# dke-lab/dgll

Hardware: AMD Instinct MI355X
Metric: aggregated edges/sec + epoch time, 3-layer GraphSAGE ogbn-products, 1/2/4/8 GPU (higher is better)
Workload: dtype bf16

## Files before the change

dgll_amd/_lib.py:

```python
import contextlib
import ctypes as C
import os

import torch

_HERE = os.path.dirname(os.path.abspath(__file__))
LIB_PATH = os.path.join(_HERE, "lib", "libdgll_hip.so")

OK = 0
F32, BF16 = 0, 1
REDUCE_SUM, REDUCE_MEAN = 0, 1
EPI_NONE, EPI_BIAS, EPI_RELU = 0, 1, 2


class BatchLoad(C.Structure):
    _fields_ = [("staged_host", C.c_void_p), ("staged_entries", C.c_int64), ("staged_dev", C.c_void_p),
                ("pos_host", C.c_void_p), ("n_outer", C.c_int64), ("pos_bytes", C.c_int), ("pos_dev", C.c_void_p),
                ("indptr", C.c_void_p), ("indices", C.c_void_p),
                ("n_hops", C.c_int), ("rows", C.c_int64 * 8), ("seeds_off", C.c_int64), ("src_off", C.c_int64 * 8), ("ptr_off", C.c_int64 * 8),
                ("cache", C.c_void_p), ("ldc", C.c_int64), ("host", C.c_void_p), ("ldh", C.c_int64), ("slot", C.c_void_p),
                ("host_map", C.c_void_p), ("feat", C.c_int), ("dtype", C.c_int), ("miss_count", C.c_void_p),
                ("feat_out", C.c_void_p * 8), ("ld_feat", C.c_int64),
                ("reduced_out", C.c_void_p), ("ld_reduced", C.c_int64), ("reduce", C.c_int),
                ("ids_out", C.c_void_p),
# ... 45 lines not shown
        _build.build()
    if not os.path.exists(LIB_PATH):
        raise ImportError("libdgll_hip.so is missing (expected at %s); run `python -m dgll_amd.build`" % LIB_PATH)
    return C.CDLL(LIB_PATH)


lib = _load()

_vp, _i32, _i64, _sz = C.c_void_p, C.c_int, C.c_int64, C.c_size_t

SIGNATURES = {
    "dgll_hip_abi_version": (_i32, []),
    "dgll_hip_last_error": (C.c_char_p, []),
    "dgll_hip_device_info": (_i32, [_i32, C.c_char_p, _i32, C.POINTER(_i32), C.POINTER(_i64)]),
    "dgll_hip_debug_tune": (_i32, [_i32, _i32]),
    "dgll_hip_debug_spmm_choice": (_i32, [_i32, _i32, _i32, _i64, _i32, _i64, _i64, _i64, _i32, _i32, _i32, _i32, _i32, _vp]),
    "dgll_hip_debug_gat_choice": (_i32, [_i32] * 17 + [_i64, _i32, _i64, _i64, _i64, _i64, _i32, _vp]),
    "dgll_hip_debug_transform_choice": (_i32, [_i32] * 12 + [_i64, _i32, _vp]),
    "dgll_hip_csr_plan_create": (_i32, [_vp, _vp, _i64, _i64, _i32, C.POINTER(_vp)]),
    "dgll_hip_csr_plan_destroy": (None, [_vp]),
    "dgll_hip_csr_plan_workspace_bytes": (_sz, [_vp, _i32]),
    "dgll_hip_csr_plan_num_long_rows": (_i64, [_vp]),
    "dgll_hip_csr_plan_num_chunks": (_i64, [_vp]),
    "dgll_hip_spmm_csr": (_i32, [_vp, _vp, _vp, _vp, _vp, _vp, _i64, _i32, _vp, _i64, _i32, _i64, _i64, _i32, _i32,
                                 _i32, _vp, _vp, _sz]),
    "dgll_hip_spmm_csr_ex": (_i32, [_vp, _vp, _vp, _vp, _vp, _vp, _i64, _i32, _vp, _i64, _i32, _i64, _i64, _i32, _i32,
                                    _i32, _vp, _vp, _sz, _vp, _i32]),
    "dgll_hip_spmm_csr_gated": (_i32, [_vp, _vp, _vp, _vp, _vp, _vp, _i64, _i32, _vp, _i64, _i32, _i64, _i64, _i32, _i32,
                                       _i32, _vp, _vp, _sz, _vp, _i32, _vp, _i64]),
    "dgll_hip_sage_fused_forward": (_i32, [_vp, _vp, _vp, _vp, _vp, _vp, _i64, _i32, _i32, _vp, _i64, _i32, _vp, _i64, _vp, _i64, _i32,
                                           _vp, _i32, _vp, _i64, _i32, _vp, _i64, _i64, _i64, _vp, _sz]),
    "dgll_hip_sddmm_csr": (_i32, [_vp, _vp, _vp, _vp, _i64, _vp, _i64, _i32, _vp, _i64, _i32]),
    "dgll_hip_gat_fwd": (_i32, [_vp, _vp, _vp, _vp, _vp, _i64, _vp, _vp, _vp, _vp, _i64, _i32, _vp, _vp, _i64, _i32, _i32,
                                C.c_float, _i32, _i32, _vp, _sz]),
    "dgll_hip_gat_fwd_ex": (_i32, [_vp, _vp, _vp, _vp, _vp, _i64, _vp, _vp, _vp, _vp, _i64, _i32, _vp, _i64, _i32, _i32,
                                   C.c_float, _i32, _vp, _sz, _i32, _i32]),
    "dgll_hip_gat_bwd_rows": (_i32, [_vp, _vp, _vp, _vp, _vp, _i64, _vp, _vp, _vp, _vp, _i64, _vp, _i64, _i32, _vp, _vp, _vp,
                                     _i64, _vp, _vp, _i64, _i32, _i32, C.c_float, _i32, _i32, _i32, _vp, _sz]),
    "dgll_hip_gat_bwd_rows_split": (_i32, [_vp, _vp, _vp, _vp, _vp, _i64, _vp, _vp, _vp, _i64, _vp, _i64, _i32, _vp, _vp, _i64, _vp, _vp,
                                           _i64, _i32, _i32, C.c_float, _i32, _i32, _vp, _vp, _sz]),
    "dgll_hip_gat_bwd_cols": (_i32, [_vp, _vp, _vp, _vp, _vp, _vp, _i64, _vp, _i64, _vp, _vp, _vp, _vp, _vp, _vp, _i64, _vp,
                                     _i32, _i64, _i32, _i32, C.c_float, _i32, _vp, _sz]),
    "dgll_hip_gat_fwd_strided": (_i32, [_vp, _vp, _vp, _vp, _vp, _i64, _vp, _vp, _i32, _vp, _i64, _i32, _vp, _i64, _i32, _i32,
                                        C.c_float, _i32, _vp, _sz]),
    "dgll_host_sampler_pool_create": (_i32, [_vp, _vp, _vp, _vp, _i64, _i64, _vp, _vp, _i32, C.c_uint64, C.c_uint64, _i32, _i32, _vp, _i64,
                                             _i64, _vp, _vp, _vp, _i32]),
# ... 206 lines not shown
```

dgll_amd/csrc/common.hpp:

```cpp
#pragma once
#include <hip/hip_runtime.h>

#include "host_common.hpp"

struct dgll_csr_plan {
    int device = 0;
    int64_t n_rows = 0, nnz = 0;
    int threshold = 256;
    int64_t n_long = 0, n_chunks = 0;
    int64_t* d_long_row = nullptr;
    int32_t* d_long_chunk0 = nullptr;
    int64_t* d_chunk_begin = nullptr;
    int64_t* d_chunk_end = nullptr;
    int64_t* d_chunk_row = nullptr;
    int flat_edges = 0;
    int64_t n_flat = 0;
    int64_t* d_flat_row0 = nullptr;
};

namespace dgll {

constexpr int kWave = 64;
constexpr int kBlock = 256;
constexpr int kWavesPerBlock = kBlock / kWave;
constexpr int kXcds = 8;

typedef uint16_t bf16_t;
typedef __attribute__((ext_vector_type(2))) __bf16 bf16x2_t;
typedef __attribute__((ext_vector_type(2))) float f32x2_t;

int hip_fail(hipError_t e, const char* what);

#define DGLL_HIP_TRY(expr)                                          \
    do {                                                            \
        hipError_t _e = (expr);                                     \
        if (_e != hipSuccess) return ::dgll::hip_fail(_e, #expr);   \
    } while (0)
// ... 106 lines not shown
```

dgll_amd/csrc/spmm.hip:

```cpp
#include <algorithm>
#include <vector>

#include "common.hpp"
#include "gat_choice.hpp"
#include "gather.hpp"
#include <type_traits>

namespace dgll {

struct LongRow { int64_t row, begin, end; };

__global__ void find_long_rows_kernel(const int64_t* __restrict__ rowptr, int64_t n_rows, int threshold,
                                      LongRow* __restrict__ out, unsigned long long* __restrict__ count,
                                      unsigned long long capacity) {
    for (int64_t r = blockIdx.x * (int64_t)blockDim.x + threadIdx.x; r < n_rows; r += (int64_t)gridDim.x * blockDim.x) {
        const int64_t b = rowptr[r], e = rowptr[r + 1];
        if (e - b > threshold) {
            const unsigned long long at = atomicAdd(count, 1ull);
            if (at < capacity) out[at] = LongRow{r, b, e};
        }
    }
}

constexpr int64_t kFlatRowCost = 4;
// ... 1 lines not shown
                                 int64_t* __restrict__ row0) {
    for (int64_t w = blockIdx.x * (int64_t)blockDim.x + threadIdx.x; w <= n_flat; w += (int64_t)gridDim.x * blockDim.x) {
        if (w == n_flat) { row0[w] = n_rows; continue; }
        const int64_t target = w * cost_per_wave;
        int64_t lo = 0, hi = n_rows;
        while (lo < hi) {
            const int64_t mid = (lo + hi) >> 1;
            if (rowptr[mid] + kFlatRowCost * mid < target) lo = mid + 1; else hi = mid;
        }
        row0[w] = lo;
    }
}

struct SpmmArgs {
    const int64_t* rowptr;
    const int32_t* col;
    const float* val;
    const void* X;
    void* Y;
    int64_t ldx, ldy, n_rows;
    int feat, reduce, epilogue;
    const float* bias;
    int threshold;
    int64_t n_chunks;
    const int64_t* chunk_begin;
    const int64_t* chunk_end;
    float* ws;
    int ws_ld;
    uint32_t chunk_blocks, row_blocks;
    int rows_per_wave;
    int flags;
    const float* row_scale;
    int accumulate;
    const void* gate;
    int64_t ldg;
    const int64_t* flat_row0;
    int64_t n_flat;
};

constexpr int kSpmmXcdRemap = 1;
constexpr int kSpmmAligned16 = 2;
constexpr int kSpmmPrefetchNext = 4;

template <typename T> __device__ __forceinline__ float load_one(const T* p);
template <> __device__ __forceinline__ float load_one<float>(const float* p) { return *p; }
template <> __device__ __forceinline__ float load_one<bf16_t>(const bf16_t* p) { return bf16_to_f32(*p); }

// ... 94 lines not shown
}

template <typename L> __device__ __forceinline__ float spmm_row_scale(const SpmmArgs& a, int64_t row, L len) {
    return a.row_scale ? a.row_scale[row] : ((a.reduce == DGLL_REDUCE_MEAN && len > 0) ? 1.0f / (float)len : 1.0f);
}

template <typename YT, int EPV, bool EXTRA, typename L>
__device__ __forceinline__ void spmm_finish_row(const SpmmArgs& a, int64_t row, L len, int c0, float (&acc)[EPV]) {
    YT* yrow = static_cast<YT*>(a.Y) + row * a.ldy;
    const bool full = c0 + EPV <= a.feat;
    RowVec<YT, EPV> prev, gatev;
    const YT* grow = nullptr;
    if constexpr (EXTRA) {
        grow = a.gate ? static_cast<const YT*>(a.gate) + row * a.ldg : nullptr;
        if (full) {
            if (a.accumulate) prev.load(yrow + c0);
            if (grow) gatev.load(grow + c0);
        }
    }
    finish_row<YT, EPV, EXTRA>(yrow, c0, a.feat, spmm_row_scale(a, row, len), a.epilogue, a.bias, acc, a.accumulate, grow, full, prev,
                               gatev);
}

template <typename XT, int EPV, int LPR, bool HAS_VAL, int U>
__device__ __forceinline__ void spmm_chunk_item(const SpmmArgs& a, const XT* __restrict__ xcol, int c0, bool col_ok, int lane, int wave,
                                                uint32_t bid) {
    const int64_t chunk = __builtin_amdgcn_readfirstlane((int)(bid * kWavesPerBlock + wave));
    if (chunk >= a.n_chunks) return;
    float acc[EPV];
#pragma unroll
    for (int i = 0; i < EPV; ++i) acc[i] = 0.0f;
    gather_edges<XT, EPV, LPR, HAS_VAL, U>(a.col, a.val, xcol, a.ldx, uniform64(a.chunk_begin[chunk]), uniform64(a.chunk_end[chunk]),
                                           lane, acc);
    if (lane < LPR && col_ok) {
        float* w = a.ws + chunk * a.ws_ld + c0;
#pragma unroll
        for (int i = 0; i < EPV; ++i) w[i] = acc[i];
    }
}

template <typename XT, typename YT, int EPV, int LPR, bool HAS_VAL, int U, bool EXTRA, bool PF = false>
__global__ __launch_bounds__(kBlock) void spmm_csr_kernel(const SpmmArgs a) {
    const int lane = lane_id();
    const int wave = __builtin_amdgcn_readfirstlane((int)(threadIdx.x >> 6));
    const int sub = lane % LPR;
    const int c0 = ((int)blockIdx.y * LPR + sub) * EPV;
    const bool col_ok = c0 < a.feat;
    const XT* xcol = static_cast<const XT*>(a.X) + (col_ok ? c0 : 0);
    uint32_t bid = blockIdx.x;

    if (bid < a.chunk_blocks) { spmm_chunk_item<XT, EPV, LPR, HAS_VAL, U>(a, xcol, c0, col_ok, lane, wave, bid); return; }

    bid -= a.chunk_blocks;
    if (a.flags & kSpmmXcdRemap) bid = xcd_remap(bid, a.row_blocks);
    const int64_t row0 = ((int64_t)bid * kWavesPerBlock + wave) * a.rows_per_wave;
    constexpr bool pf = PF;
    int64_t nb_ = 0, ne_ = 0;
    int ncol = 0;
    float nval = 0.0f;
    if (pf && row0 < a.n_rows) {
        nb_ = uniform64(a.rowptr[row0]); ne_ = uniform64(a.rowptr[row0 + 1]);
        if (nb_ + lane < ne_) {
            ncol = __builtin_nontemporal_load(a.col + nb_ + lane);
            if (HAS_VAL) nval = __builtin_nontemporal_load(a.val + nb_ + lane);
        }
    }
    for (int r = 0; r < a.rows_per_wave; ++r) {
        const int64_t row = row0 + r;
        if (row >= a.n_rows) return;
        int64_t b, e;
        int fcol = 0;
        float fval = 0.0f;
        if (pf) {
            b = nb_; e = ne_; fcol = ncol; fval = nval;
// ... 12 lines not shown
        if constexpr (EXTRA) {
            if (a.accumulate == 2 && e == b) continue;
        }
        float acc[EPV];
#pragma unroll
        for (int i = 0; i < EPV; ++i) acc[i] = 0.0f;
        gather_edges<XT, EPV, LPR, HAS_VAL, U>(a.col, a.val, xcol, a.ldx, b, e, lane, acc, pf, fcol, fval);
        if (lane < LPR && col_ok) spmm_finish_row<YT, EPV, EXTRA>(a, row, e - b, c0, acc);
    }
}

template <typename XT, typename YT, int EPV, int LPR, bool HAS_VAL, int U, bool EXTRA>
__global__ __launch_bounds__(kBlock) void spmm_csr_flat_kernel(const SpmmArgs a) {
    typedef VecIO<XT, EPV> IO;
    constexpr int SLOTS = kWave / LPR, G = SLOTS * U;
    const int lane = lane_id();
    const int wave = __builtin_amdgcn_readfirstlane((int)(threadIdx.x >> 6));
    const int sub = lane % LPR, slot = lane / LPR;
    const int c0 = ((int)blockIdx.y * LPR + sub) * EPV;
    const bool col_ok = c0 < a.feat;
    const XT* xcol = static_cast<const XT*>(a.X) + (col_ok ? c0 : 0);
    uint32_t bid = blockIdx.x;

    if (bid < a.chunk_blocks) { spmm_chunk_item<XT, EPV, LPR, HAS_VAL, U>(a, xcol, c0, col_ok, lane, wave, bid); return; }
    bid -= a.chunk_blocks;
    const int64_t w = (int64_t)bid * kWavesPerBlock + wave;
    if (w >= a.n_flat) return;
    int64_t r = uniform64(a.flat_row0[w]);
    const int64_t r_end = uniform64(a.flat_row0[w + 1]);
    if (r >= r_end) return;
    int64_t rb = uniform64(a.rowptr[r]), re = uniform64(a.rowptr[r + 1]);
    const int64_t p_end = uniform64(a.rowptr[r_end]);
    int64_t p = rb;
    const bool writer = lane < LPR && col_ok;
    const uint32_t ld32 = (uint32_t)a.ldx;
    const int thr = a.threshold;
    float acc[EPV];
#pragma unroll
    for (int i = 0; i < EPV; ++i) acc[i] = 0.0f;
    bool stop = false;

    auto flush = [&]() {
#pragma unroll
        for (int off = LPR; off < kWave; off <<= 1) {
#pragma unroll
            for (int i = 0; i < EPV; ++i) acc[i] += __shfl_xor(acc[i], off);
        }
// ... 105 lines not shown
            j += cnt;
            if (q0 + cnt == re) {
                flush();
                while (!stop && re == rb) flush();
            }
        }
        p = stop ? rb : p + j;
    }
}

template <typename XT, typename YT, int EPV, int LPR, bool HAS_VAL, bool EXTRA>
__global__ __launch_bounds__(kBlock) void spmm_rowslot_kernel(const SpmmArgs a) {
    typedef VecIO<XT, EPV> IO;
    constexpr int SLOTS = kWave / LPR;
    constexpr int U = 4;
    const int lane = lane_id();
    const int wave = __builtin_amdgcn_readfirstlane((int)(threadIdx.x >> 6));
    const int sub = lane % LPR, slot = lane / LPR;
    const int c0 = ((int)blockIdx.y * LPR + sub) * EPV;
    const bool col_ok = c0 < a.feat;
    const XT* xcol = static_cast<const XT*>(a.X) + (col_ok ? c0 : 0);
    uint32_t bid = blockIdx.x;

    if (bid < a.chunk_blocks) { spmm_chunk_item<XT, EPV, LPR, HAS_VAL, U>(a, xcol, c0, col_ok, lane, wave, bid); return; }
    bid -= a.chunk_blocks;
    const uint32_t ld32 = (uint32_t)a.ldx;
    const int64_t row0 = ((int64_t)bid * kWavesPerBlock + wave) * a.rows_per_wave;
    for (int r = 0; r < a.rows_per_wave; r += SLOTS) {
        if (row0 + r >= a.n_rows) return;
        const int64_t row = row0 + r + slot;
        int64_t b = 0, e = 0;
        if (row < a.n_rows) { b = a.rowptr[row]; e = a.rowptr[row + 1]; }
        const int64_t full_len = e - b;
        bool mine = row < a.n_rows && !(a.threshold > 0 && full_len > a.threshold);
        if constexpr (EXTRA) {
            if (a.accumulate == 2 && full_len == 0) mine = false;
        }
        const int n = mine ? (int)full_len : 0;
        float acc[EPV];
#pragma unroll
        for (int i = 0; i < EPV; ++i) acc[i] = 0.0f;
        int cnext[U];
        float wnext[U];
#pragma unroll
        for (int u = 0; u < U; ++u) {
            cnext[u] = u < n ? __builtin_nontemporal_load(a.col + b + u) : 0;
            wnext[u] = (HAS_VAL && u < n) ? __builtin_nontemporal_load(a.val + b + u) : 0.0f;
// ... 15 lines not shown
#pragma unroll
            for (int u = 0; u < U; ++u) {
                float f[EPV];
                IO::unpack(k + u < n ? v[u] : IO::zero(), f);
#pragma unroll
                for (int i = 0; i < EPV; ++i) acc[i] = HAS_VAL ? fmaf(w[u], f[i], acc[i]) : acc[i] + f[i];
            }
        }
        if (mine && col_ok) spmm_finish_row<YT, EPV, EXTRA>(a, row, n, c0, acc);
    }
}

template <typename XT, typename YT, int EPV, int LPR, int SPR, bool HAS_VAL>
__global__ __launch_bounds__(kBlock) void spmm_rowgroup_kernel(const SpmmArgs a) {
    constexpr int SLOTS = kWave / LPR, G = SLOTS / SPR, GL = kWave / G, U = 4;
    const int lane = lane_id();
    const int wave = __builtin_amdgcn_readfirstlane((int)(threadIdx.x >> 6));
    const int sub = lane % LPR, grp = lane / GL;
    const int c0 = ((int)blockIdx.y * LPR + sub) * EPV;
    const bool col_ok = c0 < a.feat;
    const XT* xcol = static_cast<const XT*>(a.X) + (col_ok ? c0 : 0);
    uint32_t bid = blockIdx.x;

    if (bid < a.chunk_blocks) { spmm_chunk_item<XT, EPV, LPR, HAS_VAL, U>(a, xcol, c0, col_ok, lane, wave, bid); return; }
    bid -= a.chunk_blocks;
    const uint32_t ld32 = (uint32_t)a.ldx;
    const bool writer = col_ok && lane % GL < LPR;
    const int64_t row0 = ((int64_t)bid * kWavesPerBlock + wave) * a.rows_per_wave;
    for (int r = 0; r < a.rows_per_wave; r += G) {
        if (row0 + r >= a.n_rows) return;
        const int64_t row = row0 + r + grp;
        int64_t b = 0, e = 0;
        if (row < a.n_rows) { b = a.rowptr[row]; e = a.rowptr[row + 1]; }
        const int64_t full_len = e - b;
        const bool mine = row < a.n_rows && !(a.threshold > 0 && full_len > a.threshold);
        const int n = mine ? (int)full_len : 0;
        float acc[EPV];
#pragma unroll
        for (int i = 0; i < EPV; ++i) acc[i] = 0.0f;
        gather_edges_grouped<XT, EPV, LPR, SPR, HAS_VAL, U>(a.col, a.val, xcol, ld32, b, n, lane, acc);
        if (mine && writer) spmm_finish_row<YT, EPV, false>(a, row, n, c0, acc);
    }
}

template <typename YT>
__global__ __launch_bounds__(kBlock) void spmm_long_finalize_kernel(const SpmmArgs a, const int64_t* __restrict__ long_row,
                                                                    const int32_t* __restrict__ long_chunk0, int64_t n_long) {
    const int lane = lane_id();
    const int64_t li = (int64_t)blockIdx.x * kWavesPerBlock + (threadIdx.x >> 6);
    if (li >= n_long) return;
    const int64_t row = long_row[li];
    const int cb = long_chunk0[li], ce = long_chunk0[li + 1];
    const float scale = spmm_row_scale(a, row, a.rowptr[row + 1] - a.rowptr[row]);
    YT* y = static_cast<YT*>(a.Y) + row * a.ldy;
    const YT* gate = a.gate ? static_cast<const YT*>(a.gate) + row * a.ldg : nullptr;
    for (int f = lane * 4; f < a.feat; f += kWave * 4) {
        float4 s = make_float4(0.f, 0.f, 0.f, 0.f);
        for (int c = cb; c < ce; c += 8) {
            float4 p[8];
#pragma unroll
            for (int u = 0; u < 8; ++u) {
                const int cc = c + u < ce ? c + u : ce - 1;
                p[u] = *reinterpret_cast<const float4*>(a.ws + (int64_t)cc * a.ws_ld + f);
            }
#pragma unroll
            for (int u = 0; u < 8; ++u)
                if (c + u < ce) { s.x += p[u].x; s.y += p[u].y; s.z += p[u].z; s.w += p[u].w; }
        }
        float v[4] = {s.x, s.y, s.z, s.w};
#pragma unroll
        for (int i = 0; i < 4; ++i) {
            if (f + i >= a.feat) continue;
            float t = v[i];
            if (a.accumulate == 1) t += load_one<YT>(y + f + i);
            t *= scale;
            if (a.epilogue & DGLL_EPI_BIAS) t += a.bias[f + i];
            if (a.epilogue & DGLL_EPI_RELU) t = fmaxf(t, 0.0f);
            if (gate && !(load_one<YT>(gate + f + i) > 0.0f)) t = 0.0f;
            if (a.accumulate == 2) t += load_one<YT>(y + f + i);
            v[i] = t;
        }
        if (f + 4 <= a.feat && (a.flags & kSpmmAligned16)) VecIO<YT, 4>::store(y + f, v);
        else
            for (int i = 0; i < 4; ++i) if (f + i < a.feat) store_one<YT>(y + f + i, v[i]);
    }
}

static int ws_ld_for(int feat) { return (feat + 7) & ~7; }

struct SpmmLaunchDesc {
    int x_dtype, y_dtype, feat;
    int64_t n_rows;
    bool has_plan;
    int64_t nnz, n_chunks, n_flat;
    bool weighted;
    int accumulate;
    bool gate, aligned16, only_long;
};

struct SpmmTune {
    int unroll = 4;
    int rows_per_wave = 0;
    int flags = 0;
    int threshold = 0;
    int rowslot = 0;
    int flat = 0;
    int flat_edges = 256;
    int rowgroup = 0;
};
static SpmmTune g_tune;

typedef dgll_spmm_choice SpmmChoice;
enum { kSpmmWaveRow = 0, kSpmmRowSlot = 1, kSpmmRowGroup = 2, kSpmmFlat = 3 };

constexpr double kRowGroupMaxAvgLen8 = 100.0, kRowGroupMaxAvgLen16 = 64.0;

static SpmmChoice spmm_choose(const SpmmLaunchDesc& d, const SpmmTune& t) {
    const bool bf = d.x_dtype == DGLL_BF16;
    SpmmChoice c{};
    c.kernel = kSpmmWaveRow;
    c.unroll = 4;
    c.epv = d.aligned16 ? (bf ? 8 : 4) : 1;
    const int vecs = (d.feat + c.epv - 1) / c.epv;
    int lpr = d.aligned16 ? 4 : 64;
    while (lpr < 64 && lpr < vecs) lpr <<= 1;
    const double avg_len = d.has_plan ? (double)d.nnz / (double)std::max<int64_t>(d.n_rows, 1) : 1e9;
    int rpw = 1;
    if (d.has_plan) {
        const double row_bytes = avg_len * d.feat * (bf ? 2.0 : 4.0);
        rpw = std::min(std::max(row_bytes > 0 ? (int)(98304.0 / row_bytes) : 8, 1), 8);
    }
// ... 150 lines not shown
        chunk0[i] = (int32_t)chunk_begin.size();
        for (int64_t b = h_list[i].begin; b < h_list[i].end; b += p->threshold) {
            chunk_begin.push_back(b);
            chunk_end.push_back(std::min<int64_t>(b + p->threshold, h_list[i].end));
            chunk_row.push_back(h_list[i].row);
        }
    }
    chunk0[h_count] = (int32_t)chunk_begin.size();
    p->n_long = (int64_t)h_count;
    p->n_chunks = (int64_t)chunk_begin.size();
    if (p->n_long > 0) {
        PLAN_TRY(hipMalloc(&p->d_long_row, sizeof(int64_t) * h_count));
        PLAN_TRY(hipMalloc(&p->d_long_chunk0, sizeof(int32_t) * (h_count + 1)));
        PLAN_TRY(hipMalloc(&p->d_chunk_begin, sizeof(int64_t) * chunk_begin.size()));
        PLAN_TRY(hipMalloc(&p->d_chunk_end, sizeof(int64_t) * chunk_end.size()));
        PLAN_TRY(hipMalloc(&p->d_chunk_row, sizeof(int64_t) * chunk_row.size()));
        PLAN_TRY(hipMemcpyAsync(p->d_chunk_row, chunk_row.data(), sizeof(int64_t) * chunk_row.size(), hipMemcpyHostToDevice, s));
        PLAN_TRY(hipMemcpyAsync(p->d_long_row, long_row.data(), sizeof(int64_t) * h_count, hipMemcpyHostToDevice, s));
        PLAN_TRY(hipMemcpyAsync(p->d_long_chunk0, chunk0.data(), sizeof(int32_t) * (h_count + 1), hipMemcpyHostToDevice, s));
        PLAN_TRY(hipMemcpyAsync(p->d_chunk_begin, chunk_begin.data(), sizeof(int64_t) * chunk_begin.size(), hipMemcpyHostToDevice, s));
        PLAN_TRY(hipMemcpyAsync(p->d_chunk_end, chunk_end.data(), sizeof(int64_t) * chunk_end.size(), hipMemcpyHostToDevice, s));
        PLAN_TRY(hipStreamSynchronize(s));
    }
    if (n_rows > 0 && g_tune.flat_edges > 0) {
        p->flat_edges = g_tune.flat_edges;
        p->n_flat = (nnz + kFlatRowCost * n_rows + p->flat_edges - 1) / p->flat_edges;
        PLAN_TRY(hipMalloc(&p->d_flat_row0, sizeof(int64_t) * (size_t)(p->n_flat + 1)));
        const int blocks = (int)std::min<int64_t>((p->n_flat + 1 + kBlock - 1) / kBlock, 4096);
        hipLaunchKernelGGL(flat_row0_kernel, dim3(blocks), dim3(kBlock), 0, s, rowptr, n_rows, (int64_t)p->flat_edges, p->n_flat,
                           p->d_flat_row0);
        PLAN_TRY(hipGetLastError());
        PLAN_TRY(hipStreamSynchronize(s));
    }
#undef PLAN_TRY
    cleanup();
    *out_plan = p;
    return DGLL_OK;
}

extern int g_tune_mfma_kperm;
extern int g_tune_res_per_cu;
extern int g_tune_res_grid_cap;
extern int g_tune_loader_blocks_per_cu;

DGLL_API int dgll_hip_debug_tune(int key, int value) {
    switch (key) {
        case 0: g_tune.unroll = value; break;
        case 1: g_tune.rows_per_wave = value; break;
        case 2: g_tune.flags = value; break;
        case 3: g_tune.threshold = value; break;
        case 4: g_tune_mfma_kperm = value; break;
        case 5: g_tune.rowslot = value; break;
        case 13: g_tune.flat = value; break;
        case 14: g_tune.flat_edges = value; break;
        case 15: g_tune.rowgroup = value; break;
        case 7: break;
        case 9: g_gat_tune.gen = value; break;
        case 11: g_tune_res_per_cu = value; break;
        case 12: g_tune_loader_blocks_per_cu = value; break;
        case 16: g_tune_res_grid_cap = value; break;
        default: set_error("unknown tuning key"); return DGLL_ERR_INVALID;
    }
    return DGLL_OK;
}

DGLL_API int dgll_hip_debug_spmm_choice(int x_dtype, int y_dtype, int feat, int64_t n_rows, int has_plan, int64_t nnz, int64_t n_chunks,
                                        int64_t n_flat, int weighted, int accumulate, int gate, int aligned16, int only_long,
                                        dgll_spmm_choice* out) {
    DGLL_REQUIRE(out != nullptr, "out is NULL");
    DGLL_REQUIRE((x_dtype == DGLL_F32 || x_dtype == DGLL_BF16) && (y_dtype == DGLL_F32 || y_dtype == DGLL_BF16), "dtype");
    DGLL_REQUIRE(feat > 0 && n_rows > 0 && nnz >= 0 && n_chunks >= 0 && n_flat >= 0, "bad launch description");
    const bool plan = has_plan != 0;
    *out = spmm_choose(SpmmLaunchDesc{x_dtype, y_dtype, feat, n_rows, plan, plan ? nnz : 0, plan ? n_chunks : 0, plan ? n_flat : 0,
                                      weighted != 0, accumulate, gate != 0, aligned16 != 0, only_long != 0}, g_tune);
    return DGLL_OK;
}

DGLL_API void dgll_hip_csr_plan_destroy(dgll_csr_plan* p) {
    if (!p) return;
    if (p->d_long_row) (void)hipFree(p->d_long_row);
    if (p->d_long_chunk0) (void)hipFree(p->d_long_chunk0);
    if (p->d_chunk_begin) (void)hipFree(p->d_chunk_begin);
    if (p->d_chunk_end) (void)hipFree(p->d_chunk_end);
    if (p->d_chunk_row) (void)hipFree(p->d_chunk_row);
    if (p->d_flat_row0) (void)hipFree(p->d_flat_row0);
    delete p;
}

DGLL_API size_t dgll_hip_csr_plan_workspace_bytes(const dgll_csr_plan* p, int feat) {
    if (!p || p->n_chunks == 0 || feat <= 0) return 0;
    return (size_t)p->n_chunks * (size_t)ws_ld_for(feat) * sizeof(float);
}

DGLL_API int64_t dgll_hip_csr_plan_num_long_rows(const dgll_csr_plan* p) { return p ? p->n_long : 0; }
DGLL_API int64_t dgll_hip_csr_plan_num_chunks(const dgll_csr_plan* p) { return p ? p->n_chunks : 0; }


DGLL_API int dgll_hip_spmm_csr(void* stream, const dgll_csr_plan* plan, const int64_t* rowptr, const int32_t* col,
                               const float* val, const void* X, int64_t ldx, int x_dtype, void* Y, int64_t ldy,
                               int y_dtype, int64_t n_rows, int64_t n_cols, int feat, int reduce, int epilogue,
                               const float* bias, void* workspace, size_t workspace_bytes) {
    return dgll_spmm_csr_impl(stream, plan, rowptr, col, val, X, ldx, x_dtype, Y, ldy, y_dtype, n_rows, n_cols, feat, reduce,
                              epilogue, bias, workspace, workspace_bytes, nullptr, 0, nullptr, 0, 0);
}

DGLL_API int dgll_hip_spmm_csr_ex(void* stream, const dgll_csr_plan* plan, const int64_t* rowptr, const int32_t* col,
                                  const float* val, const void* X, int64_t ldx, int x_dtype, void* Y, int64_t ldy,
                                  int y_dtype, int64_t n_rows, int64_t n_cols, int feat, int reduce, int epilogue,
                                  const float* bias, void* workspace, size_t workspace_bytes, const float* row_scale,
                                  int accumulate) {
    return dgll_spmm_csr_impl(stream, plan, rowptr, col, val, X, ldx, x_dtype, Y, ldy, y_dtype, n_rows, n_cols, feat, reduce,
                              epilogue, bias, workspace, workspace_bytes, row_scale, accumulate, nullptr, 0, 0);
}

DGLL_API int dgll_hip_spmm_csr_gated(void* stream, const dgll_csr_plan* plan, const int64_t* rowptr, const int32_t* col,
                                     const float* val, const void* X, int64_t ldx, int x_dtype, void* Y, int64_t ldy,
                                     int y_dtype, int64_t n_rows, int64_t n_cols, int feat, int reduce, int epilogue,
                                     const float* bias, void* workspace, size_t workspace_bytes, const float* row_scale,
// ... 14 lines not shown
    if (n_rows == 0 || feat == 0) return DGLL_OK;
    DGLL_REQUIRE(rowptr && X && Y, "NULL rowptr/X/Y");
    DGLL_REQUIRE(ldx >= feat && ldy >= feat, "leading dimension smaller than feat");
    DGLL_REQUIRE(ldx < ((int64_t)1 << 31) && n_cols < ((int64_t)1 << 31), "leading dimension / column count must fit 31 bits");
    DGLL_REQUIRE(x_dtype == DGLL_F32 || x_dtype == DGLL_BF16, "x_dtype");
    DGLL_REQUIRE(y_dtype == DGLL_F32 || y_dtype == DGLL_BF16, "y_dtype");
    DGLL_REQUIRE(reduce == DGLL_REDUCE_SUM || reduce == DGLL_REDUCE_MEAN, "reduce");
    DGLL_REQUIRE((epilogue & ~(DGLL_EPI_BIAS | DGLL_EPI_RELU)) == 0, "epilogue");
    DGLL_REQUIRE(!(epilogue & DGLL_EPI_BIAS) || bias, "DGLL_EPI_BIAS needs bias");
    if (x_dtype == DGLL_F32 && y_dtype == DGLL_BF16) {
        set_error("fp32 input with bf16 output is not supported");
        return DGLL_ERR_UNSUPPORTED;
    }
    hipStream_t s = static_cast<hipStream_t>(stream);

    SpmmArgs a{};
    a.rowptr = rowptr; a.col = col; a.val = val; a.X = X; a.Y = Y;
    a.ldx = ldx; a.ldy = ldy; a.n_rows = n_rows; a.feat = feat; a.reduce = reduce; a.epilogue = epilogue; a.bias = bias;
    a.ws_ld = ws_ld_for(feat);
    a.flags = g_tune.flags;
    a.row_scale = row_scale;
    a.accumulate = accumulate;
    a.gate = gate; a.ldg = ldg;
    if (plan) {
        DGLL_REQUIRE(plan->n_rows == n_rows, "plan was built for a different CSR");
        a.threshold = plan->threshold;
        a.n_chunks = plan->n_chunks;
        a.chunk_begin = plan->d_chunk_begin;
        a.chunk_end = plan->d_chunk_end;
        if (plan->n_chunks > 0) {
            const size_t need = dgll_hip_csr_plan_workspace_bytes(plan, feat);
            if (!workspace || workspace_bytes < need) {
                set_error("workspace too small for the plan's long-row partials");
                return DGLL_ERR_WORKSPACE;
            }
            a.ws = static_cast<float*>(workspace);
        }
    }
    if (only_long && (!plan || plan->n_long == 0)) return DGLL_OK;
    const int esz = x_dtype == DGLL_BF16 ? 2 : 4;
    const int ysz = y_dtype == DGLL_BF16 ? 2 : 4;
    const bool fast = aligned16(X) && aligned16(Y) && (ldx * esz) % 16 == 0 && (ldy * ysz) % 16 == 0 &&
                      (!gate || (aligned16(gate) && (ldg * ysz) % 16 == 0));
    if (fast) a.flags |= kSpmmAligned16;

    const SpmmLaunchDesc d{x_dtype, y_dtype, feat, n_rows, plan != nullptr, plan ? plan->nnz : 0, plan ? plan->n_chunks : 0,
                           plan && plan->d_flat_row0 ? plan->n_flat : 0, val != nullptr, accumulate, gate != nullptr, fast,
                           only_long != 0};
    const SpmmChoice c = spmm_choose(d, g_tune);
    DGLL_REQUIRE(c.row_blocks + c.chunk_blocks < (int64_t)0x7fffffff, "grid too large");
    a.rows_per_wave = c.rows_per_wave;
    a.row_blocks = (uint32_t)c.row_blocks;
    a.chunk_blocks = (uint32_t)c.chunk_blocks;
    if (c.kernel == kSpmmFlat) { a.flat_row0 = plan->d_flat_row0; a.n_flat = plan->n_flat; }
    hipError_t err = spmm_launch(d, c, a, s);
    if (err != hipSuccess) return hip_fail(err, "spmm_csr_kernel launch");

    if (plan && plan->n_long > 0) {
        dim3 grid((uint32_t)((plan->n_long + kWavesPerBlock - 1) / kWavesPerBlock));
        if (y_dtype == DGLL_F32)
            hipLaunchKernelGGL(spmm_long_finalize_kernel<float>, grid, dim3(kBlock), 0, s, a, plan->d_long_row,
                               plan->d_long_chunk0, plan->n_long);
        else
            hipLaunchKernelGGL(spmm_long_finalize_kernel<bf16_t>, grid, dim3(kBlock), 0, s, a, plan->d_long_row,
                               plan->d_long_chunk0, plan->n_long);
        err = hipGetLastError();
        if (err != hipSuccess) return hip_fail(err, "spmm_long_finalize_kernel launch");
    }
    return DGLL_OK;
}
```

include/dgll_hip.h:

```cpp
#ifndef DGLL_HIP_H
#define DGLL_HIP_H

#include <stddef.h>
#include <stdint.h>

#ifdef __cplusplus
extern "C" {
#endif

#define DGLL_HIP_ABI_VERSION 1

enum { DGLL_OK = 0, DGLL_ERR_INVALID = -1, DGLL_ERR_HIP = -2, DGLL_ERR_UNSUPPORTED = -3, DGLL_ERR_WORKSPACE = -4 };
enum { DGLL_F32 = 0, DGLL_BF16 = 1 };
enum { DGLL_REDUCE_SUM = 0, DGLL_REDUCE_MEAN = 1 };
enum { DGLL_EPI_NONE = 0, DGLL_EPI_BIAS = 1, DGLL_EPI_RELU = 2 };

typedef struct dgll_csr_plan dgll_csr_plan;

int dgll_hip_abi_version(void);
const char* dgll_hip_last_error(void);
int dgll_hip_device_info(int device, char* name, int name_len, int* compute_units, int64_t* global_mem_bytes);

int dgll_hip_debug_tune(int key, int value);

// ... 11 lines not shown
    const char* message;
};
int dgll_hip_debug_gat_choice(int pass, int dtype, int heads, int fo, int mode, int edge_scale, int rowscore, int drop, int phase,
                              int t_stride, int t_aligned16, int dd_aligned16, int sd_out, int score_epilogue,
                              int score_behind_row, int score_pitch_equal, int second_follows, int64_t pad_bytes, int has_plan,
                              int64_t n_rows, int64_t nnz, int64_t n_chunks, int64_t n_long, int y_aligned,
                              struct dgll_gat_choice* out);

struct dgll_transform_choice {
    int kernel, nt, ntw, nc, cs, colsplit, epi, dual, rows_per_block, lds_bytes, per_cu, bits_in_epilogue, error;
    int64_t workgroups, row_sequences, n_blocks;
    const char* message;
};
int dgll_hip_debug_transform_choice(int N, int K1, int K2, int mask, int out_f32, int row_scale, int addend, int out_gate,
                                    int gate_bits, int out_aligned, int ldw_equal, int dual, int64_t M, int n_cu,
                                    struct dgll_transform_choice* out);

int dgll_hip_csr_plan_create(void* stream, const int64_t* rowptr, int64_t n_rows, int64_t nnz,
                             int long_row_threshold, dgll_csr_plan** out_plan);
void dgll_hip_csr_plan_destroy(dgll_csr_plan* plan);
size_t dgll_hip_csr_plan_workspace_bytes(const dgll_csr_plan* plan, int feat);
int64_t dgll_hip_csr_plan_num_long_rows(const dgll_csr_plan* plan);
int64_t dgll_hip_csr_plan_num_chunks(const dgll_csr_plan* plan);

int dgll_hip_spmm_csr(void* stream, const dgll_csr_plan* plan,
                      const int64_t* rowptr, const int32_t* col, const float* val,
                      const void* X, int64_t ldx, int x_dtype,
                      void* Y, int64_t ldy, int y_dtype,
                      int64_t n_rows, int64_t n_cols, int feat,
                      int reduce, int epilogue, const float* bias,
                      void* workspace, size_t workspace_bytes);

int dgll_hip_spmm_csr_ex(void* stream, const dgll_csr_plan* plan,
                         const int64_t* rowptr, const int32_t* col, const float* val,
                         const void* X, int64_t ldx, int x_dtype, void* Y, int64_t ldy, int y_dtype,
                         int64_t n_rows, int64_t n_cols, int feat, int reduce, int epilogue, const float* bias,
                         void* workspace, size_t workspace_bytes, const float* row_scale, int accumulate);

int dgll_hip_spmm_csr_gated(void* stream, const dgll_csr_plan* plan,
                            const int64_t* rowptr, const int32_t* col, const float* val,
                            const void* X, int64_t ldx, int x_dtype, void* Y, int64_t ldy, int y_dtype,
                            int64_t n_rows, int64_t n_cols, int feat, int reduce, int epilogue, const float* bias,
                            void* workspace, size_t workspace_bytes, const float* row_scale, int accumulate,
                            const void* gate, int64_t ldg);

int dgll_hip_sddmm_csr(void* stream, const int64_t* rowptr, const int32_t* col,
// ... 371 lines not shown
```

Measured before the change: 32.88 billion.

## Reduce small long-row chunks in-block via LDS; batch finalize per row

Long rows that split into at most four chunks are now packed by the plan into shared blocks. Each wave gathers one chunk and the block sums the partials in LDS and applies the epilogue directly, with no workspace write and no finalize pass. Rows with more chunks still go to the finalize kernel, now launched as one block per row, where all four waves fetch partials in batches through LDS. This adds plan-build host work, extra device arrays and __syncthreads on the chunk path, all meant to remove workspace round-trips and finalize launch work.

```diff
diff --git a/dgll_amd/_lib.py b/dgll_amd/_lib.py
--- a/dgll_amd/_lib.py
+++ b/dgll_amd/_lib.py
@@ -91,6 +91,9 @@
     "dgll_hip_csr_plan_workspace_bytes": (_sz, [_vp, _i32]),
     "dgll_hip_csr_plan_num_long_rows": (_i64, [_vp]),
     "dgll_hip_csr_plan_num_chunks": (_i64, [_vp]),
+    "dgll_hip_csr_plan_num_spread_rows": (_i64, [_vp]),
+    "dgll_hip_csr_plan_num_inblock_blocks": (_i64, [_vp]),
+    "dgll_hip_debug_spmm_long_pack": (_i32, [_vp, _i64, _i64, C.POINTER(_i64), C.POINTER(_i64), _vp, _vp, _vp, _vp, _vp, _vp]),
     "dgll_hip_spmm_csr": (_i32, [_vp, _vp, _vp, _vp, _vp, _vp, _i64, _i32, _vp, _i64, _i32, _i64, _i64, _i32, _i32,
                                  _i32, _vp, _vp, _sz]),
     "dgll_hip_spmm_csr_ex": (_i32, [_vp, _vp, _vp, _vp, _vp, _vp, _i64, _i32, _vp, _i64, _i32, _i64, _i64, _i32, _i32,
diff --git a/dgll_amd/csrc/common.hpp b/dgll_amd/csrc/common.hpp
--- a/dgll_amd/csrc/common.hpp
+++ b/dgll_amd/csrc/common.hpp
@@ -13,6 +13,12 @@
     int64_t* d_chunk_begin = nullptr;
     int64_t* d_chunk_end = nullptr;
     int64_t* d_chunk_row = nullptr;
+    int64_t n_ib_blocks = 0, n_spread = 0, n_spread_chunks = 0;
+    int64_t n_items = 0;
+    int64_t* d_item_begin = nullptr;
+    int64_t* d_item_end = nullptr;
+    int64_t* d_spread_row = nullptr;
+    int32_t* d_spread_chunk0 = nullptr;
     int flat_edges = 0;
     int64_t n_flat = 0;
     int64_t* d_flat_row0 = nullptr;
diff --git a/dgll_amd/csrc/spmm.hip b/dgll_amd/csrc/spmm.hip
--- a/dgll_amd/csrc/spmm.hip
+++ b/dgll_amd/csrc/spmm.hip
@@ -47,7 +47,7 @@
     int feat, reduce, epilogue;
     const float* bias;
     int threshold;
-    int64_t n_chunks;
+    uint32_t n_items, ib_blocks;
     const int64_t* chunk_begin;
     const int64_t* chunk_end;
     float* ws;
@@ -188,20 +188,80 @@
                                gatev);
 }
 
-template <typename XT, int EPV, int LPR, bool HAS_VAL, int U>
-__device__ __forceinline__ void spmm_chunk_item(const SpmmArgs& a, const XT* __restrict__ xcol, int c0, bool col_ok, int lane, int wave,
-                                                uint32_t bid) {
-    const int64_t chunk = __builtin_amdgcn_readfirstlane((int)(bid * kWavesPerBlock + wave));
-    if (chunk >= a.n_chunks) return;
+template <typename YT>
+__device__ __forceinline__ void spmm_long_epilogue(const SpmmArgs& a, YT* __restrict__ y, const YT* __restrict__ gate, float scale, int f,
+                                                   const float4& s) {
+    float v[4] = {s.x, s.y, s.z, s.w};
+#pragma unroll
+    for (int i = 0; i < 4; ++i) {
+        if (f + i >= a.feat) continue;
+        float t = v[i];
+        if (a.accumulate == 1) t += load_one<YT>(y + f + i);
+        t *= scale;
+        if (a.epilogue & DGLL_EPI_BIAS) t += a.bias[f + i];
+        if (a.epilogue & DGLL_EPI_RELU) t = fmaxf(t, 0.0f);
+        if (gate && !(load_one<YT>(gate + f + i) > 0.0f)) t = 0.0f;
+        if (a.accumulate == 2) t += load_one<YT>(y + f + i);
+        v[i] = t;
+    }
+    if (f + 4 <= a.feat && (a.flags & kSpmmAligned16)) VecIO<YT, 4>::store(y + f, v);
+    else
+        for (int i = 0; i < 4; ++i) if (f + i < a.feat) store_one<YT>(y + f + i, v[i]);
+}
+
+template <typename XT, typename YT, int EPV, int LPR, bool HAS_VAL, int U>
+__device__ __forceinline__ void spmm_chunk_phase(int wave, uint32_t bid) {
+    constexpr int W = LPR * EPV;
+    static_assert(W % 4 == 0 && W <= 8 * kWave, "in-block item: float4 reads of the partials");
+    __shared__ __attribute__((aligned(16))) float part[kWavesPerBlock][W];
+    typedef const __attribute__((address_space(4))) SpmmArgs* KernArgs;
+    KernArgs ap = (KernArgs)__builtin_amdgcn_kernarg_segment_ptr();
+    asm volatile("" : "+s"(ap));
+    const SpmmArgs& a = *(const SpmmArgs*)ap;
+    const int lane = (int)__lane_id();
+    const int c0 = ((int)blockIdx.y * LPR + lane % LPR) * EPV;
+    const bool col_ok = c0 < a.feat;
+    const XT* xcol = static_cast<const XT*>(a.X) + (col_ok ? c0 : 0);
+
+    const bool inblock = bid < a.ib_blocks;
+    const uint32_t item = __builtin_amdgcn_readfirstlane(bid * kWavesPerBlock + wave);
+    if (!inblock && item >= a.n_items) return;
+    const int64_t b = uniform64(a.chunk_begin[item]), e = uniform64(a.chunk_end[item]);
     float acc[EPV];
 #pragma unroll
     for (int i = 0; i < EPV; ++i) acc[i] = 0.0f;
-    gather_edges<XT, EPV, LPR, HAS_VAL, U>(a.col, a.val, xcol, a.ldx, uniform64(a.chunk_begin[chunk]), uniform64(a.chunk_end[chunk]),
-                                           lane, acc);
-    if (lane < LPR && col_ok) {
-        float* w = a.ws + chunk * a.ws_ld + c0;
-#pragma unroll
-        for (int i = 0; i < EPV; ++i) w[i] = acc[i];
+    gather_edges<XT, EPV, LPR, HAS_VAL, U>(a.col, a.val, xcol, a.ldx, b, e, lane, acc);
+    if (!inblock) {
+        if (lane < LPR && col_ok) {
+            float* w = a.ws + (int64_t)(item - a.ib_blocks * kWavesPerBlock) * a.ws_ld + c0;
+#pragma unroll
+            for (int i = 0; i < EPV; ++i) w[i] = acc[i];
+        }
+        return;
+    }
+    if (lane < LPR) {
+#pragma unroll
+        for (int i = 0; i < EPV; ++i) part[wave][lane * EPV + i] = acc[i];
+    }
+    __syncthreads();
+    const int64_t row = uniform64(a.chunk_end[(int64_t)a.n_items + item]);
+    if (row < 0) return;
+    const int slots = __builtin_amdgcn_readfirstlane((int)a.chunk_begin[(int64_t)a.n_items + item]);
+    const int s0 = slots & 0xff, ns = slots >> 8;
+    const float scale = spmm_row_scale(a, row, a.rowptr[row + 1] - a.rowptr[row]);
+    YT* y = static_cast<YT*>(a.Y) + row * a.ldy;
+    const YT* gate = a.gate ? static_cast<const YT*>(a.gate) + row * a.ldg : nullptr;
+#pragma unroll 1
+    for (int j = lane * 4; j < W; j += kWave * 4) {
+        const int f = (int)blockIdx.y * W + j;
+        if (f >= a.feat) return;
+        float4 s = make_float4(0.f, 0.f, 0.f, 0.f);
+#pragma unroll 1
+        for (int k = 0; k < ns; ++k) {
+            const float4 p = *reinterpret_cast<const float4*>(&part[s0 + k][j]);
+            s.x += p.x; s.y += p.y; s.z += p.z; s.w += p.w;
+        }
+        spmm_long_epilogue<YT>(a, y, gate, scale, f, s);
     }
 }
 
@@ -215,7 +275,7 @@
     const XT* xcol = static_cast<const XT*>(a.X) + (col_ok ? c0 : 0);
     uint32_t bid = blockIdx.x;
 
-    if (bid < a.chunk_blocks) { spmm_chunk_item<XT, EPV, LPR, HAS_VAL, U>(a, xcol, c0, col_ok, lane, wave, bid); return; }
+    if (bid < a.chunk_blocks) { spmm_chunk_phase<XT, YT, EPV, LPR, HAS_VAL, U>(wave, bid); return; }
 
     bid -= a.chunk_blocks;
     if (a.flags & kSpmmXcdRemap) bid = xcd_remap(bid, a.row_blocks);
@@ -274,7 +334,7 @@
     const XT* xcol = static_cast<const XT*>(a.X) + (col_ok ? c0 : 0);
     uint32_t bid = blockIdx.x;
 
-    if (bid < a.chunk_blocks) { spmm_chunk_item<XT, EPV, LPR, HAS_VAL, U>(a, xcol, c0, col_ok, lane, wave, bid); return; }
+    if (bid < a.chunk_blocks) { spmm_chunk_phase<XT, YT, EPV, LPR, HAS_VAL, U>(wave, bid); return; }
     bid -= a.chunk_blocks;
     const int64_t w = (int64_t)bid * kWavesPerBlock + wave;
     if (w >= a.n_flat) return;
@@ -426,7 +486,7 @@
     const XT* xcol = static_cast<const XT*>(a.X) + (col_ok ? c0 : 0);
     uint32_t bid = blockIdx.x;
 
-    if (bid < a.chunk_blocks) { spmm_chunk_item<XT, EPV, LPR, HAS_VAL, U>(a, xcol, c0, col_ok, lane, wave, bid); return; }
+    if (bid < a.chunk_blocks) { spmm_chunk_phase<XT, YT, EPV, LPR, HAS_VAL, U>(wave, bid); return; }
     bid -= a.chunk_blocks;
     const uint32_t ld32 = (uint32_t)a.ldx;
     const int64_t row0 = ((int64_t)bid * kWavesPerBlock + wave) * a.rows_per_wave;
@@ -488,7 +548,7 @@
     const XT* xcol = static_cast<const XT*>(a.X) + (col_ok ? c0 : 0);
     uint32_t bid = blockIdx.x;
 
-    if (bid < a.chunk_blocks) { spmm_chunk_item<XT, EPV, LPR, HAS_VAL, U>(a, xcol, c0, col_ok, lane, wave, bid); return; }
+    if (bid < a.chunk_blocks) { spmm_chunk_phase<XT, YT, EPV, LPR, HAS_VAL, U>(wave, bid); return; }
     bid -= a.chunk_blocks;
     const uint32_t ld32 = (uint32_t)a.ldx;
     const bool writer = col_ok && lane % GL < LPR;
@@ -509,50 +569,86 @@
     }
 }
 
+constexpr int kFinBatch = 32;
 template <typename YT>
 __global__ __launch_bounds__(kBlock) void spmm_long_finalize_kernel(const SpmmArgs a, const int64_t* __restrict__ long_row,
                                                                     const int32_t* __restrict__ long_chunk0, int64_t n_long) {
+    constexpr int PER = kFinBatch / kWavesPerBlock;
+    __shared__ __attribute__((aligned(16))) float part[kFinBatch][4 * kWave];
     const int lane = lane_id();
-    const int64_t li = (int64_t)blockIdx.x * kWavesPerBlock + (threadIdx.x >> 6);
+    const int wave = __builtin_amdgcn_readfirstlane((int)(threadIdx.x >> 6));
+    const int64_t li = blockIdx.x;
     if (li >= n_long) return;
-    const int64_t row = long_row[li];
-    const int cb = long_chunk0[li], ce = long_chunk0[li + 1];
+    const int64_t row = uniform64(long_row[li]);
+    const int cb = __builtin_amdgcn_readfirstlane(long_chunk0[li]), ce = __builtin_amdgcn_readfirstlane(long_chunk0[li + 1]);
     const float scale = spmm_row_scale(a, row, a.rowptr[row + 1] - a.rowptr[row]);
     YT* y = static_cast<YT*>(a.Y) + row * a.ldy;
     const YT* gate = a.gate ? static_cast<const YT*>(a.gate) + row * a.ldg : nullptr;
-    for (int f = lane * 4; f < a.feat; f += kWave * 4) {
+    for (int f0 = 0; f0 < a.feat; f0 += kWave * 4) {
+        const int f = f0 + lane * 4;
+        const bool live = f < a.feat;
+        float4 p[PER];
+        auto fetch = [&](int c) {
+#pragma unroll
+            for (int u = 0; u < PER; ++u) {
+                const int cc = c + u * kWavesPerBlock + wave;
+                p[u] = live ? *reinterpret_cast<const float4*>(a.ws + (int64_t)(cc < ce ? cc : ce - 1) * a.ws_ld + f)
+                            : make_float4(0.f, 0.f, 0.f, 0.f);
+            }
+        };
         float4 s = make_float4(0.f, 0.f, 0.f, 0.f);
-        for (int c = cb; c < ce; c += 8) {
-            float4 p[8];
-#pragma unroll
-            for (int u = 0; u < 8; ++u) {
-                const int cc = c + u < ce ? c + u : ce - 1;
-                p[u] = *reinterpret_cast<const float4*>(a.ws + (int64_t)cc * a.ws_ld + f);
-            }
-#pragma unroll
-            for (int u = 0; u < 8; ++u)
-                if (c + u < ce) { s.x += p[u].x; s.y += p[u].y; s.z += p[u].z; s.w += p[u].w; }
-        }
-        float v[4] = {s.x, s.y, s.z, s.w};
-#pragma unroll
-        for (int i = 0; i < 4; ++i) {
-            if (f + i >= a.feat) continue;
-            float t = v[i];
-            if (a.accumulate == 1) t += load_one<YT>(y + f + i);
-            t *= scale;
-            if (a.epilogue & DGLL_EPI_BIAS) t += a.bias[f + i];
-            if (a.epilogue & DGLL_EPI_RELU) t = fmaxf(t, 0.0f);
-            if (gate && !(load_one<YT>(gate + f + i) > 0.0f)) t = 0.0f;
-            if (a.accumulate == 2) t += load_one<YT>(y + f + i);
-            v[i] = t;
-        }
-        if (f + 4 <= a.feat && (a.flags & kSpmmAligned16)) VecIO<YT, 4>::store(y + f, v);
-        else
-            for (int i = 0; i < 4; ++i) if (f + i < a.feat) store_one<YT>(y + f + i, v[i]);
+        fetch(cb);
+        for (int c = cb; c < ce; c += kFinBatch) {
+#pragma unroll
+            for (int u = 0; u < PER; ++u) *reinterpret_cast<float4*>(&part[u * kWavesPerBlock + wave][lane * 4]) = p[u];
+            if (c + kFinBatch < ce) fetch(c + kFinBatch);
+            __syncthreads();
+            if (wave == 0) {
+                const int n = ce - c < kFinBatch ? ce - c : kFinBatch;
+                for (int k = 0; k < n; ++k) {
+                    const float4 q = *reinterpret_cast<const float4*>(&part[k][lane * 4]);
+                    s.x += q.x; s.y += q.y; s.z += q.z; s.w += q.w;
+                }
+            }
+            __syncthreads();
+        }
+        if (wave == 0 && live) spmm_long_epilogue<YT>(a, y, gate, scale, f, s);
     }
 }
 
 static int ws_ld_for(int feat) { return (feat + 7) & ~7; }
+
+struct SpmmLongPack {
+    int64_t n_blocks = 0;
+    std::vector<int32_t> slot_row, slot_chunk;
+    std::vector<int32_t> block_row, block_first, block_count;
+    std::vector<int32_t> spread;
+};
+static void spmm_pack_long_rows(const int32_t* counts, int64_t n, SpmmLongPack& out) {
+    out = SpmmLongPack();
+    int used = kWavesPerBlock, rows = 0;
+    for (int64_t i = 0; i < n; ++i) {
+        const int c = counts[i];
+        if (c > kWavesPerBlock) { out.spread.push_back((int32_t)i); continue; }
+        if (c <= 0) continue;
+        if (used + c > kWavesPerBlock) {
+            ++out.n_blocks;
+            used = rows = 0;
+            out.slot_row.resize(out.n_blocks * kWavesPerBlock, -1);
+            out.slot_chunk.resize(out.n_blocks * kWavesPerBlock, 0);
+            out.block_row.resize(out.n_blocks * kWavesPerBlock, -1);
+            out.block_first.resize(out.n_blocks * kWavesPerBlock, 0);
+            out.block_count.resize(out.n_blocks * kWavesPerBlock, 0);
+        }
+        const int64_t base = (out.n_blocks - 1) * kWavesPerBlock;
+        for (int k = 0; k < c; ++k) { out.slot_row[base + used + k] = (int32_t)i; out.slot_chunk[base + used + k] = k; }
+        out.block_row[base + rows] = (int32_t)i;
+        out.block_first[base + rows] = used;
+        out.block_count[base + rows] = c;
+        used += c;
+        ++rows;
+    }
+}
 
 struct SpmmLaunchDesc {
     int x_dtype, y_dtype, feat;
@@ -573,6 +669,7 @@
     int flat = 0;
     int flat_edges = 256;
     int rowgroup = 0;
+    int long_inblock = 0;
 };
 static SpmmTune g_tune;
 
@@ -769,6 +866,52 @@
         PLAN_TRY(hipMemcpyAsync(p->d_chunk_end, chunk_end.data(), sizeof(int64_t) * chunk_end.size(), hipMemcpyHostToDevice, s));
         PLAN_TRY(hipStreamSynchronize(s));
     }
+    if (p->n_long > 0) {
+        std::vector<int32_t> counts(h_count);
+        for (size_t i = 0; i < h_count; ++i) counts[i] = chunk0[i + 1] - chunk0[i];
+        SpmmLongPack pk;
+        spmm_pack_long_rows(counts.data(), (int64_t)h_count, pk);
+        const size_t n_slots = (size_t)pk.n_blocks * kWavesPerBlock;
+        std::vector<int64_t> item_begin(n_slots, 0), item_end(n_slots, 0);
+        for (size_t i = 0; i < n_slots; ++i) {
+            if (pk.slot_row[i] < 0) continue;
+            const int32_t c = chunk0[pk.slot_row[i]] + pk.slot_chunk[i];
+            item_begin[i] = chunk_begin[c];
+            item_end[i] = chunk_end[c];
+        }
+        std::vector<int64_t> sp_row(pk.spread.size());
+        std::vector<int32_t> sp_chunk0(pk.spread.size() + 1, 0);
+        for (size_t i = 0; i < pk.spread.size(); ++i) {
+            const int32_t r = pk.spread[i];
+            sp_row[i] = long_row[r];
+            sp_chunk0[i] = (int32_t)(item_begin.size() - n_slots);
+            item_begin.insert(item_begin.end(), chunk_begin.begin() + chunk0[r], chunk_begin.begin() + chunk0[r + 1]);
+            item_end.insert(item_end.end(), chunk_end.begin() + chunk0[r], chunk_end.begin() + chunk0[r + 1]);
+        }
+        sp_chunk0[pk.spread.size()] = (int32_t)(item_begin.size() - n_slots);
+        p->n_ib_blocks = pk.n_blocks;
+        p->n_spread = (int64_t)pk.spread.size();
+        p->n_spread_chunks = (int64_t)(item_begin.size() - n_slots);
+        p->n_items = (int64_t)item_begin.size();
+        for (size_t i = 0; i < n_slots; ++i) {
+            const bool own = pk.block_row[i] >= 0;
+            item_begin.push_back(own ? (int64_t)(pk.block_first[i] | (pk.block_count[i] << 8)) : 0);
+            item_end.push_back(own ? long_row[pk.block_row[i]] : -1);
+        }
+        auto upload = [&](auto** dst, const auto& v) -> hipError_t {
+            if (v.empty()) return hipSuccess;
+            hipError_t r = hipMalloc(dst, sizeof(v[0]) * v.size());
+            if (r != hipSuccess) return r;
+            return hipMemcpyAsync(*dst, v.data(), sizeof(v[0]) * v.size(), hipMemcpyHostToDevice, s);
+        };
+        PLAN_TRY(upload(&p->d_item_begin, item_begin));
+        PLAN_TRY(upload(&p->d_item_end, item_end));
+        if (p->n_spread > 0) {
+            PLAN_TRY(upload(&p->d_spread_row, sp_row));
+            PLAN_TRY(upload(&p->d_spread_chunk0, sp_chunk0));
+        }
+        PLAN_TRY(hipStreamSynchronize(s));
+    }
     if (n_rows > 0 && g_tune.flat_edges > 0) {
         p->flat_edges = g_tune.flat_edges;
         p->n_flat = (nnz + kFlatRowCost * n_rows + p->flat_edges - 1) / p->flat_edges;
@@ -801,6 +944,7 @@
         case 13: g_tune.flat = value; break;
         case 14: g_tune.flat_edges = value; break;
         case 15: g_tune.rowgroup = value; break;
+        case 18: g_tune.long_inblock = value; break;
         case 7: break;
         case 9: g_gat_tune.gen = value; break;
         case 11: g_tune_res_per_cu = value; break;
@@ -830,6 +974,10 @@
     if (p->d_chunk_begin) (void)hipFree(p->d_chunk_begin);
     if (p->d_chunk_end) (void)hipFree(p->d_chunk_end);
     if (p->d_chunk_row) (void)hipFree(p->d_chunk_row);
+    if (p->d_item_begin) (void)hipFree(p->d_item_begin);
+    if (p->d_item_end) (void)hipFree(p->d_item_end);
+    if (p->d_spread_row) (void)hipFree(p->d_spread_row);
+    if (p->d_spread_chunk0) (void)hipFree(p->d_spread_chunk0);
     if (p->d_flat_row0) (void)hipFree(p->d_flat_row0);
     delete p;
 }
@@ -841,6 +989,31 @@
 
 DGLL_API int64_t dgll_hip_csr_plan_num_long_rows(const dgll_csr_plan* p) { return p ? p->n_long : 0; }
 DGLL_API int64_t dgll_hip_csr_plan_num_chunks(const dgll_csr_plan* p) { return p ? p->n_chunks : 0; }
+DGLL_API int64_t dgll_hip_csr_plan_num_spread_rows(const dgll_csr_plan* p) { return p ? p->n_spread : 0; }
+DGLL_API int64_t dgll_hip_csr_plan_num_inblock_blocks(const dgll_csr_plan* p) { return p ? p->n_ib_blocks : 0; }
+
+DGLL_API int dgll_hip_debug_spmm_long_pack(const int32_t* chunk_counts, int64_t n_long, int64_t capacity, int64_t* n_blocks,
+                                           int64_t* n_spread, int32_t* slot_row, int32_t* slot_chunk, int32_t* block_row,
+                                           int32_t* block_first, int32_t* block_count, int32_t* spread) {
+    DGLL_REQUIRE(n_long >= 0 && (chunk_counts != nullptr || n_long == 0), "bad chunk counts");
+    DGLL_REQUIRE(n_blocks != nullptr && n_spread != nullptr && capacity >= 0, "bad output arguments");
+    for (int64_t i = 0; i < n_long; ++i) DGLL_REQUIRE(chunk_counts[i] >= 1, "a long row has at least one chunk");
+    SpmmLongPack pk;
+    spmm_pack_long_rows(chunk_counts, n_long, pk);
+    *n_blocks = pk.n_blocks;
+    *n_spread = (int64_t)pk.spread.size();
+    const int64_t n_slots = pk.n_blocks * kWavesPerBlock;
+    if (capacity == 0) return DGLL_OK;
+    DGLL_REQUIRE(capacity >= n_slots && capacity >= (int64_t)pk.spread.size(), "capacity too small for the schedule");
+    DGLL_REQUIRE(slot_row && slot_chunk && block_row && block_first && block_count && spread, "NULL output array");
+    std::copy(pk.slot_row.begin(), pk.slot_row.end(), slot_row);
+    std::copy(pk.slot_chunk.begin(), pk.slot_chunk.end(), slot_chunk);
+    std::copy(pk.block_row.begin(), pk.block_row.end(), block_row);
+    std::copy(pk.block_first.begin(), pk.block_first.end(), block_first);
+    std::copy(pk.block_count.begin(), pk.block_count.end(), block_count);
+    std::copy(pk.spread.begin(), pk.spread.end(), spread);
+    return DGLL_OK;
+}
 
 
 DGLL_API int dgll_hip_spmm_csr(void* stream, const dgll_csr_plan* plan, const int64_t* rowptr, const int32_t* col,
@@ -901,12 +1074,22 @@
     a.row_scale = row_scale;
     a.accumulate = accumulate;
     a.gate = gate; a.ldg = ldg;
+    const bool inblock = g_tune.long_inblock != 1;
     if (plan) {
         DGLL_REQUIRE(plan->n_rows == n_rows, "plan was built for a different CSR");
         a.threshold = plan->threshold;
-        a.n_chunks = plan->n_chunks;
-        a.chunk_begin = plan->d_chunk_begin;
-        a.chunk_end = plan->d_chunk_end;
+        if (inblock) {
+            DGLL_REQUIRE(plan->n_items < (int64_t)0x7fffffff, "too many chunk items");
+            a.ib_blocks = (uint32_t)plan->n_ib_blocks;
+            a.n_items = (uint32_t)plan->n_items;
+            a.chunk_begin = plan->d_item_begin;
+            a.chunk_end = plan->d_item_end;
+        } else {
+            DGLL_REQUIRE(plan->n_chunks < (int64_t)0x7fffffff, "too many chunk items");
+            a.n_items = (uint32_t)plan->n_chunks;
+            a.chunk_begin = plan->d_chunk_begin;
+            a.chunk_end = plan->d_chunk_end;
+        }
         if (plan->n_chunks > 0) {
             const size_t need = dgll_hip_csr_plan_workspace_bytes(plan, feat);
             if (!workspace || workspace_bytes < need) {
@@ -923,7 +1106,7 @@
                       (!gate || (aligned16(gate) && (ldg * ysz) % 16 == 0));
     if (fast) a.flags |= kSpmmAligned16;
 
-    const SpmmLaunchDesc d{x_dtype, y_dtype, feat, n_rows, plan != nullptr, plan ? plan->nnz : 0, plan ? plan->n_chunks : 0,
+    const SpmmLaunchDesc d{x_dtype, y_dtype, feat, n_rows, plan != nullptr, plan ? plan->nnz : 0, (int64_t)a.n_items,
                            plan && plan->d_flat_row0 ? plan->n_flat : 0, val != nullptr, accumulate, gate != nullptr, fast,
                            only_long != 0};
     const SpmmChoice c = spmm_choose(d, g_tune);
@@ -935,14 +1118,16 @@
     hipError_t err = spmm_launch(d, c, a, s);
     if (err != hipSuccess) return hip_fail(err, "spmm_csr_kernel launch");
 
-    if (plan && plan->n_long > 0) {
-        dim3 grid((uint32_t)((plan->n_long + kWavesPerBlock - 1) / kWavesPerBlock));
+    const int64_t n_fin = !plan ? 0 : (inblock ? plan->n_spread : plan->n_long);
+    if (n_fin > 0) {
+        DGLL_REQUIRE(n_fin < (int64_t)0x7fffffff, "grid too large");
+        const int64_t* fin_row = inblock ? plan->d_spread_row : plan->d_long_row;
+        const int32_t* fin_chunk0 = inblock ? plan->d_spread_chunk0 : plan->d_long_chunk0;
+        dim3 grid((uint32_t)n_fin);
         if (y_dtype == DGLL_F32)
-            hipLaunchKernelGGL(spmm_long_finalize_kernel<float>, grid, dim3(kBlock), 0, s, a, plan->d_long_row,
-                               plan->d_long_chunk0, plan->n_long);
+            hipLaunchKernelGGL(spmm_long_finalize_kernel<float>, grid, dim3(kBlock), 0, s, a, fin_row, fin_chunk0, n_fin);
         else
-            hipLaunchKernelGGL(spmm_long_finalize_kernel<bf16_t>, grid, dim3(kBlock), 0, s, a, plan->d_long_row,
-                               plan->d_long_chunk0, plan->n_long);
+            hipLaunchKernelGGL(spmm_long_finalize_kernel<bf16_t>, grid, dim3(kBlock), 0, s, a, fin_row, fin_chunk0, n_fin);
         err = hipGetLastError();
         if (err != hipSuccess) return hip_fail(err, "spmm_long_finalize_kernel launch");
     }
diff --git a/include/dgll_hip.h b/include/dgll_hip.h
--- a/include/dgll_hip.h
+++ b/include/dgll_hip.h
@@ -57,6 +57,11 @@
 size_t dgll_hip_csr_plan_workspace_bytes(const dgll_csr_plan* plan, int feat);
 int64_t dgll_hip_csr_plan_num_long_rows(const dgll_csr_plan* plan);
 int64_t dgll_hip_csr_plan_num_chunks(const dgll_csr_plan* plan);
+int64_t dgll_hip_csr_plan_num_spread_rows(const dgll_csr_plan* plan);
+int64_t dgll_hip_csr_plan_num_inblock_blocks(const dgll_csr_plan* plan);
+int dgll_hip_debug_spmm_long_pack(const int32_t* chunk_counts, int64_t n_long, int64_t capacity, int64_t* n_blocks,
+                                  int64_t* n_spread, int32_t* slot_row, int32_t* slot_chunk, int32_t* block_row,
+                                  int32_t* block_first, int32_t* block_count, int32_t* spread);
 
 int dgll_hip_spmm_csr(void* stream, const dgll_csr_plan* plan,
                       const int64_t* rowptr, const int32_t* col, const float* val,
```

Result: no change. 32.62 billion (-0.8%).
